# DecaYale/SYN3R

Measured on AMD Instinct MI355X. Metric: llff_3view_train_loop_iters_per_sec, higher is better.
Workload: dtype f32 raster / f16 UNet (f32 accumulate); 1 GPU; LLFF fern-like 3-view block: 50 raster fwd+bwd iters (l1 loss) (200000 Gaussians, 1920x1080, SH3) + 1 SVD (step,pass): CFG UNet fwd [2,14,8,72,128] f16 + fused Euler step; frames=14, parallelism=scene-parallel x1

## Files before the change

### syn3r_amd/csrc/raster_bin.hip

```cpp
#include "common.h"
#include "raster_common.h"

using namespace syn3r;

namespace syn3r {

size_t binning_bytes(long long P) {
    size_t n = (size_t)(P > 0 ? P : 1);
    return 2 * align256(n * 8) + 2 * align256(n * 4) + sort_scratch_bytes(n) + 256;
}

BinningState carve_binning(void* buf, long long P) {
    size_t n = (size_t)(P > 0 ? P : 1);
    char* p = (char*)buf;
    BinningState b;
    b.keys_a = (unsigned long long*)p; p += align256(n * 8);
    b.keys_b = (unsigned long long*)p; p += align256(n * 8);
    b.vals_a = (unsigned*)p; p += align256(n * 4);
    b.vals_b = (unsigned*)p; p += align256(n * 4);
    b.sort_scratch = p;
    return b;
}

}

namespace {

__global__ void __launch_bounds__(256) k_dup_tiles(int N, const unsigned* __restrict__ order,
                                                   const float* __restrict__ means2D, const int* __restrict__ radii,
                                                   const unsigned* __restrict__ offsets, int gx, int gy,
                                                   unsigned* __restrict__ keys, unsigned* __restrict__ vals,
                                                   unsigned cap, unsigned* __restrict__ header,
                                                   uint2* __restrict__ ranges, int tiles) {
    const int i = blockIdx.x * 256 + threadIdx.x;
    for (int t = i; t < tiles; t += gridDim.x * 256) ranges[t] = make_uint2(0u, 0u);
    const int lane = threadIdx.x & 63;
    const bool valid = i < N;
    unsigned id = valid ? order[i] : 0u;
    int r = valid ? radii[id] : 0;
    int x0 = 0, y0 = 0, x1 = 0, y1 = 0;
    if (r > 0) tile_rect(means2D[2 * (size_t)id], means2D[2 * (size_t)id + 1], r, gx, gy, x0, y0, x1, y1);
    const int w = x1 - x0;
    const unsigned cnt = (unsigned)(w * (y1 - y0));
    const unsigned incl = wave_scan_incl(cnt);
    const unsigned local = incl - cnt;
    const unsigned total = __shfl(incl, 63, 64);
    const int first = blockIdx.x * 256 + (threadIdx.x & ~63);
    const unsigned base = first < N ? offsets[first] : 0u;
    const float inv_w = w > 0 ? 1.0f / (float)w : 0.0f;
    for (unsigned t = 0; t < total; t += 64) {
        const unsigned p = t + lane;
        int j = 0;
#pragma unroll
        for (int step = 32; step > 0; step >>= 1) {
            unsigned lc = __shfl(local, j + step, 64);
            if (lc <= p) j += step;
        }
        const unsigned k = p - __shfl(local, j, 64);
        const int xj = __shfl(x0, j, 64), yj = __shfl(y0, j, 64), wj = __shfl(w, j, 64);
        const float iwj = __shfl(inv_w, j, 64);
        const unsigned idj = __shfl(id, j, 64);
        if (p < total) {
            const int ty = (int)(((float)k + 0.5f) * iwj);
            int tyc = ty;
            if ((unsigned)(tyc * wj) > k) --tyc;
            else if ((unsigned)((tyc + 1) * wj) <= k) ++tyc;
            const int tx = (int)k - tyc * wj;
            const unsigned o = base + p;
            if (o < cap) {
                keys[o] = (unsigned)((yj + tyc) * gx + xj + tx);
                vals[o] = idj;
            } else {
                header[1] = 1u;
            }
        }
    }
}

__global__ void __launch_bounds__(256) k_tile_ranges(long long P_cap, const unsigned* __restrict__ header,
                                                     const unsigned* __restrict__ keys,
                                                     uint2* __restrict__ ranges) {
    long long P = (long long)header[0];
    if (P > P_cap) P = P_cap;
    long long i = (long long)blockIdx.x * 256 + threadIdx.x;
    if (i >= P) return;
    unsigned cur = keys[i];
    if (i == 0) ranges[cur].x = 0;
    else {
        unsigned prev = keys[i - 1];
        if (cur != prev) {
            ranges[prev].y = (unsigned)i;
            ranges[cur].x = (unsigned)i;
        }
    }
    if (i == P - 1) ranges[cur].y = (unsigned)P;
}

constexpr int kBinThreads = 512;
constexpr int kOffThreads = 1024;
#ifndef SYN3R_MAX_SUPER
#define SYN3R_MAX_SUPER 512
#endif
constexpr int kMaxSuper = SYN3R_MAX_SUPER;

struct BinPlan { int ss, sgx, sgy, nsuper, rounds, nchunks; bool ok; };
inline BinPlan bin_plan(int N, int gx, int gy) {
    BinPlan b;
    for (b.ss = 0; b.ss <= 3; ++b.ss) {
        const int side = 1 << b.ss;
        b.sgx = (gx + side - 1) / side; b.sgy = (gy + side - 1) / side;
        b.nsuper = b.sgx * b.sgy;
        if (b.nsuper <= kMaxSuper) break;
    }
    if (b.ss > 3) b.ss = 3;
    b.ok = b.nsuper <= kMaxSuper;
    const int max_chunks = b.ok ? (int)(kBinCounters / (size_t)b.nsuper) : 1;
    const int units = (N + kBinThreads - 1) / kBinThreads;
    b.rounds = (units + max_chunks - 1) / max_chunks;
    if (b.rounds < 1) b.rounds = 1;
    b.nchunks = (units + b.rounds - 1) / b.rounds;
    return b;
}

inline bool hier_binning(int N, int gx, int gy) {
    static const int on = tune_env("SYN3R_BIN_HIER", 1);
    return on != 0 && bin_plan(N, gx, gy).ok;
}

struct BinRect { int x0, y0, x1, y1; };
__device__ __forceinline__ BinRect bin_rect(int i, int N, const float* __restrict__ means2D, const int* __restrict__ radii, int gx, int gy) {
    BinRect r; r.x0 = r.y0 = r.x1 = r.y1 = 0;
    if (i < N) {
        const int rad = radii[i];
        if (rad > 0) tile_rect(means2D[2 * (size_t)i], means2D[2 * (size_t)i + 1], rad, gx, gy, r.x0, r.y0, r.x1, r.y1);
    }
    return r;
}
__device__ __forceinline__ unsigned short clip_rect(const BinRect& q, int sx, int sy, int ss) {
    const int bx = sx << ss, by = sy << ss, side = 1 << ss;
    const int rx0 = max(q.x0 - bx, 0), rx1 = min(q.x1 - bx, side), ry0 = max(q.y0 - by, 0), ry1 = min(q.y1 - by, side);
    return (unsigned short)(rx0 | (rx1 << 4) | (ry0 << 8) | (ry1 << 12));
}

__global__ void __launch_bounds__(kBinThreads) k_super_count(int N, const float* __restrict__ means2D, const int* __restrict__ radii,
                                                             int gx, int gy, int ss, int sgx, int nsuper, int rounds, int nchunks,
                                                             unsigned* __restrict__ counters, unsigned* __restrict__ header) {
    __shared__ unsigned tot[kMaxSuper];
    for (int s = threadIdx.x; s < nsuper; s += kBinThreads) tot[s] = 0u;
    __syncthreads();
    int pairs = 0;
    for (int r = 0; r < rounds; ++r) {
        const int i = (blockIdx.x * rounds + r) * kBinThreads + threadIdx.x;
        const BinRect q = bin_rect(i, N, means2D, radii, gx, gy);
        if (q.x1 > q.x0 && q.y1 > q.y0) {
            pairs += (q.x1 - q.x0) * (q.y1 - q.y0);
            const int side1 = (1 << ss) - 1, sx0 = q.x0 >> ss, sx1 = (q.x1 + side1) >> ss, sy0 = q.y0 >> ss, sy1 = (q.y1 + side1) >> ss;
            for (int sy = sy0; sy < sy1; ++sy)
                for (int sx = sx0; sx < sx1; ++sx) atomicAdd(&tot[sy * sgx + sx], 1u);
        }
    }
    __syncthreads();
    for (int s = threadIdx.x; s < nsuper; s += kBinThreads) counters[(size_t)blockIdx.x * nsuper + s] = tot[s];
    __shared__ unsigned pairs_s;
    if (threadIdx.x == 0) pairs_s = 0u;
    __syncthreads();
    pairs = wave_sum_i(pairs);
    if ((threadIdx.x & 63) == 0 && pairs) atomicAdd(&pairs_s, (unsigned)pairs);
    __syncthreads();
    if (threadIdx.x == 0 && pairs_s) atomicAdd(&header[3], pairs_s);
}

__global__ void __launch_bounds__(kBinThreads) k_super_append(int N, const float* __restrict__ depths, const float* __restrict__ means2D,
                                                              const int* __restrict__ radii, int gx, int gy, int ss, int sgx, int nsuper,
                                                              int rounds, int nchunks, const unsigned* __restrict__ counters,
                                                              unsigned* __restrict__ sstart, unsigned cap,
                                                              unsigned long long* __restrict__ skeys, unsigned* __restrict__ header) {
    __shared__ unsigned run[kMaxSuper];
    __shared__ unsigned tot_s[kMaxSuper], pre_s[kMaxSuper];
    __shared__ unsigned part_tot[kMaxSuper > kBinThreads ? kMaxSuper : kBinThreads], part_pre[kMaxSuper > kBinThreads ? kMaxSuper : kBinThreads];
    const int lane = threadIdx.x & 63, wv = threadIdx.x >> 6;
    {
        const int PARTS = max(1, min(8, kBinThreads / nsuper));
        const int per = (nchunks + PARTS - 1) / PARTS;
        for (int w = threadIdx.x; w < nsuper * PARTS; w += kBinThreads) {
            const int s_ = w % nsuper, part = w / nsuper;
            const int c0 = part * per, c1 = min(nchunks, c0 + per);
            unsigned tot = 0, pre = 0;
            constexpr int UN = 32;
            for (int cb = c0; cb < c1; cb += UN) {
                unsigned c[UN];
#pragma unroll
                for (int u = 0; u < UN; ++u) c[u] = cb + u < c1 ? counters[(size_t)(cb + u) * nsuper + s_] : 0u;
#pragma unroll
                for (int u = 0; u < UN; ++u) { tot += c[u]; pre += cb + u < (int)blockIdx.x ? c[u] : 0u; }
            }
            part_tot[w] = tot; part_pre[w] = pre;
        }
        __syncthreads();
        for (int s_ = threadIdx.x; s_ < nsuper; s_ += kBinThreads) {
            unsigned tot = 0, pre = 0;
            for (int k = 0; k < PARTS; ++k) { tot += part_tot[k * nsuper + s_]; pre += part_pre[k * nsuper + s_]; }
            tot_s[s_] = tot; pre_s[s_] = pre;
        }
        __syncthreads();
        if (wv == 0) {
            constexpr int PER = kMaxSuper / 64;
            unsigned c[PER], sum = 0;
#pragma unroll
            for (int k = 0; k < PER; ++k) { const int s_ = lane * PER + k; c[k] = s_ < nsuper ? tot_s[s_] : 0u; sum += c[k]; }
            const unsigned incl = wave_scan_incl(sum);
            unsigned ex = incl - sum;
#pragma unroll
            for (int k = 0; k < PER; ++k) {
                const int s_ = lane * PER + k;
                if (s_ < nsuper) {
                    run[s_] = ex + pre_s[s_];
                    if (blockIdx.x == 0) sstart[s_] = ex;
                }
                ex += c[k];
            }
            if (blockIdx.x == 0 && lane == 63) { sstart[nsuper] = incl; header[2] = incl; }
        }
        __syncthreads();
    }
    for (int r = 0; r < rounds; ++r) {
        const int i = (blockIdx.x * rounds + r) * kBinThreads + threadIdx.x;
        const BinRect q = bin_rect(i, N, means2D, radii, gx, gy);
        if (q.x1 > q.x0 && q.y1 > q.y0) {
            const unsigned long long key = ((unsigned long long)__float_as_uint(depths[i]) << 32) | (unsigned)i;
            const int side1 = (1 << ss) - 1, sx0 = q.x0 >> ss, sx1 = (q.x1 + side1) >> ss, sy0 = q.y0 >> ss, sy1 = (q.y1 + side1) >> ss;
            for (int sy = sy0; sy < sy1; ++sy)
                for (int sx = sx0; sx < sx1; ++sx) {
                    const unsigned o = atomicAdd(&run[sy * sgx + sx], 1u);
                    if (o < cap) skeys[o] = key;
                    else header[1] = 1u;
                }
        }
    }
}

__device__ __forceinline__ void super_range(int s, const unsigned* __restrict__ sstart, unsigned cap, unsigned& b, unsigned& e) {
    b = min(sstart[s], cap); e = min(sstart[s + 1], cap);
}

constexpr int kSortLds = 4096;
constexpr int kSuperSortThreads = 1024;
__device__ __forceinline__ void cmpx(unsigned long long& a, unsigned long long& b) { if (a > b) { const unsigned long long t = a; a = b; b = t; } }
__device__ __forceinline__ int pair_lo(int t, int j) { return (t << 1) - (t & (j - 1)); }
__device__ __forceinline__ void bitonic_dists(unsigned long long* buf, int m, int j) {
    for (; j >= 2; j >>= 2) {
        const int jh = j >> 1;
        for (int t = threadIdx.x; t < (m >> 2); t += kSuperSortThreads) {
            const int e0 = pair_lo(pair_lo(t, jh), j);
            unsigned long long a = buf[e0], b = buf[e0 + jh], c = buf[e0 + j], d = buf[e0 + j + jh];
            cmpx(a, c); cmpx(b, d);
            cmpx(a, b); cmpx(c, d);
            buf[e0] = a; buf[e0 + jh] = b; buf[e0 + j] = c; buf[e0 + j + jh] = d;
        }
        __syncthreads();
    }
    if (j == 1) {
        for (int t = threadIdx.x; t < (m >> 1); t += kSuperSortThreads) cmpx(buf[2 * t], buf[2 * t + 1]);
        __syncthreads();
    }
}
__device__ __forceinline__ void bitonic_merge(unsigned long long* buf, int m, int k) {
    if (k == 2) {
        for (int t = threadIdx.x; t < (m >> 1); t += kSuperSortThreads) cmpx(buf[2 * t], buf[2 * t + 1]);
        __syncthreads();
        return;
    }
    const int q = k >> 2;
    for (int t = threadIdx.x; t < (m >> 2); t += kSuperSortThreads) {
        const int off = t & (q - 1), blk = (t - off) << 2;
        const int ia = blk + off, ib = ia + q, ird = blk + (k - 1 - off), irc = ird - q;
        unsigned long long a = buf[ia], b = buf[ib], c = buf[irc], d = buf[ird];
        cmpx(a, d); cmpx(b, c);
        cmpx(a, b); cmpx(c, d);
        buf[ia] = a; buf[ib] = b; buf[irc] = c; buf[ird] = d;
    }
    __syncthreads();
    bitonic_dists(buf, m, q >> 1);
}

__device__ __forceinline__ bool rect_has(unsigned r, int rx, int ry) {
    return rx >= (int)(r & 15u) && rx < (int)((r >> 4) & 15u) && ry >= (int)((r >> 8) & 15u) && ry < (int)(r >> 12);
}

constexpr int kBinUnroll = 8;
__device__ __forceinline__ void tile_quarter(unsigned b, unsigned e, int q, unsigned& qb, unsigned& qe) {
    const unsigned len = (e - b + 3u) / 4u;
    qb = min(e, b + (unsigned)q * len); qe = min(e, qb + len);
}

__device__ __forceinline__ void super_tile_counts(int sx, int sy, int ss, int gx, int gy, unsigned n, const unsigned short* srect_b,
                                                  unsigned* __restrict__ tcount) {
    const int lane = threadIdx.x & 63, wv = threadIdx.x >> 6, side = 1 << ss;
    const unsigned len = (n + 3u) / 4u;
    for (int it = wv; it < side * side * 4; it += kSuperSortThreads / 64) {
        const int ti = it >> 2, q = it & 3;
        const int rx = ti & (side - 1), ry = ti >> ss;
        const int tx = (sx << ss) + rx, ty = (sy << ss) + ry;
        if (tx >= gx || ty >= gy) continue;
        const unsigned lo = min(n, (unsigned)q * len), hi = min(n, lo + len);
        unsigned cnt = 0;
        for (unsigned i0 = lo; i0 < hi; i0 += 256) {
            unsigned short r[4];
#pragma unroll
            for (int u = 0; u < 4; ++u) r[u] = srect_b[min(i0 + u * 64 + lane, hi - 1u)];
#pragma unroll
            for (int u = 0; u < 4; ++u) cnt += (i0 + u * 64 + lane < hi && rect_has(r[u], rx, ry)) ? 1u : 0u;
        }
#pragma unroll
        for (int o = 32; o > 0; o >>= 1) cnt += __shfl_xor(cnt, o, 64);
        if (lane == 0) tcount[4 * ((size_t)ty * gx + tx) + q] = cnt;
    }
}

__global__ void __launch_bounds__(kSuperSortThreads, 8) k_super_sort(int N, const float* __restrict__ means2D, const int* __restrict__ radii,
                                                                  int gx, int gy, int ss, int sgx, const unsigned* __restrict__ sstart, unsigned cap,
                                                                  unsigned long long* __restrict__ skeys, unsigned* __restrict__ sid,
                                                                  unsigned short* __restrict__ srect, unsigned* __restrict__ tcount) {
    extern __shared__ __attribute__((aligned(16))) unsigned long long sk[];
    const int s_ = blockIdx.x, sx = s_ % sgx, sy = s_ / sgx;
    unsigned b, e;
    super_range(s_, sstart, cap, b, e);
    const int n = (int)(e - b);
    if (n == 0) { super_tile_counts(sx, sy, ss, gx, gy, 0u, srect, tcount); return; }
    unsigned long long* gk = skeys + b;
    const unsigned long long INF = ~0ull;
    int m = 1;
    while (m < n) m <<= 1;
    const unsigned long long* sorted;
    if (m <= kSortLds) {
        for (int i = threadIdx.x; i < m; i += kSuperSortThreads) sk[i] = i < n ? gk[i] : INF;
        __syncthreads();
        for (int k = 2; k <= m; k <<= 1) bitonic_merge(sk, m, k);
        sorted = sk;
    } else {
        for (int p0 = 0; p0 < n; p0 += kSortLds) {
            for (int i = threadIdx.x; i < kSortLds; i += kSuperSortThreads) sk[i] = p0 + i < n ? gk[p0 + i] : INF;
            __syncthreads();
            for (int k = 2; k <= kSortLds; k <<= 1) bitonic_merge(sk, kSortLds, k);
            for (int i = threadIdx.x; i < kSortLds; i += kSuperSortThreads) if (p0 + i < n) gk[p0 + i] = sk[i];
            __syncthreads();
        }
        for (int k = kSortLds << 1; k <= m; k <<= 1) {
            const int h = k >> 1;
            for (int t = threadIdx.x; t < (m >> 1); t += kSuperSortThreads) {
                const int off = t & (h - 1), l = pair_lo(t, h), r = l - off + (k - 1 - off);
                if (r < n) { unsigned long long a = gk[l], c = gk[r]; if (a > c) { gk[l] = c; gk[r] = a; } }
            }
            __syncthreads();
            for (int j = k >> 2; j >= kSortLds; j >>= 1) {
                for (int t = threadIdx.x; t < (m >> 1); t += kSuperSortThreads) {
                    const int l = pair_lo(t, j), r = l + j;
                    if (r < n) { unsigned long long a = gk[l], c = gk[r]; if (a > c) { gk[l] = c; gk[r] = a; } }
                }
                __syncthreads();
            }
            for (int p0 = 0; p0 < n; p0 += kSortLds) {
                for (int i = threadIdx.x; i < kSortLds; i += kSuperSortThreads) sk[i] = p0 + i < n ? gk[p0 + i] : INF;
                __syncthreads();
                bitonic_dists(sk, kSortLds, kSortLds >> 1);
                for (int i = threadIdx.x; i < kSortLds; i += kSuperSortThreads) if (p0 + i < n) gk[p0 + i] = sk[i];
                __syncthreads();
            }
        }
        sorted = gk;
    }
    if (sorted == sk) {
        unsigned short clip[kSortLds / kSuperSortThreads];
#pragma unroll
        for (int u = 0; u < kSortLds / kSuperSortThreads; ++u) {
            const int i = threadIdx.x + u * kSuperSortThreads;
            clip[u] = 0;
            if (i < n) {
                const unsigned id = (unsigned)sk[i];
                const BinRect q = bin_rect((int)id, N, means2D, radii, gx, gy);
                clip[u] = clip_rect(q, sx, sy, ss);
                sid[b + i] = id;
                srect[b + i] = clip[u];
            }
        }
        __syncthreads();
        unsigned short* sr = (unsigned short*)sk;
#pragma unroll
        for (int u = 0; u < kSortLds / kSuperSortThreads; ++u) {
            const int i = threadIdx.x + u * kSuperSortThreads;
            if (i < n) sr[i] = clip[u];
        }
        __syncthreads();
        super_tile_counts(sx, sy, ss, gx, gy, (unsigned)n, sr, tcount);
        return;
    }
    for (int i = threadIdx.x; i < n; i += kSuperSortThreads) {
        const unsigned id = (unsigned)sorted[i];
        const BinRect q = bin_rect((int)id, N, means2D, radii, gx, gy);
        sid[b + i] = id;
        srect[b + i] = clip_rect(q, sx, sy, ss);
    }
    __syncthreads();
    super_tile_counts(sx, sy, ss, gx, gy, (unsigned)n, srect + b, tcount);
}

__global__ void __launch_bounds__(kOffThreads) k_tile_offsets(int tiles, const unsigned* __restrict__ tcount, unsigned cap,
                                                              uint2* __restrict__ ranges, unsigned* __restrict__ header,
                                                              unsigned* __restrict__ tile_order) {
    __shared__ unsigned smem[kOffThreads / 64 + 1];
    __shared__ unsigned bh[256];
    if (tile_order) { for (int k = threadIdx.x; k < 256; k += kOffThreads) bh[k] = 0u; __syncthreads(); }
    constexpr int PER = 8;
    unsigned carry = 0;
    for (int start = 0; start < tiles; start += kOffThreads * PER) {
        const int t0 = start + threadIdx.x * PER;
        unsigned c[PER], sum = 0;
#pragma unroll
        for (int k = 0; k < PER; ++k) {
            c[k] = 0u;
            if (t0 + k < tiles) { const uint4 q4 = ((const uint4*)tcount)[t0 + k]; c[k] = (q4.x + q4.y) + (q4.z + q4.w); }
            sum += c[k];
        }
        unsigned total;
        unsigned ex = block_exclusive_scan<kOffThreads / 64>(sum, smem, total) + carry;
#pragma unroll
        for (int k = 0; k < PER; ++k) {
            if (t0 + k < tiles) ranges[t0 + k] = c[k] ? make_uint2(min(ex, cap), min(ex + c[k], cap)) : make_uint2(0u, 0u);
            if (tile_order && t0 + k < tiles) atomicAdd(&bh[255u - min(255u, c[k] >> 5)], 1u);
            ex += c[k];
        }
        carry += total;
    }
    if (tile_order) {
        __syncthreads();
        if (threadIdx.x < 64) {
            const int l = threadIdx.x;
            unsigned c[4], sum = 0;
#pragma unroll
            for (int k = 0; k < 4; ++k) { c[k] = bh[4 * l + k]; sum += c[k]; }
            unsigned ex = wave_scan_incl(sum) - sum;
#pragma unroll
            for (int k = 0; k < 4; ++k) { bh[4 * l + k] = ex; ex += c[k]; }
        }
        __syncthreads();
        for (int t = threadIdx.x; t < tiles; t += kOffThreads) {
            const uint4 q4 = ((const uint4*)tcount)[t];
            const unsigned c = (q4.x + q4.y) + (q4.z + q4.w);
            tile_order[atomicAdd(&bh[255u - min(255u, c >> 5)], 1u)] = (unsigned)t;
        }
    }
    if (threadIdx.x == 0) {
        const bool over = carry > cap || header[2] > cap;
        header[0] = over ? max(carry, max(header[3], header[2])) : carry;
        if (over) header[1] = 1u;
    }
}

__global__ void __launch_bounds__(256) k_tile_write(int gx, int tiles, int ss, int sgx, const unsigned* __restrict__ sstart, unsigned cap,
                                                    const unsigned* __restrict__ sid, const unsigned short* __restrict__ srect,
                                                    const uint2* __restrict__ ranges, const unsigned* __restrict__ tcount,
                                                    unsigned* __restrict__ point_list) {
    const int t = blockIdx.x, q = threadIdx.x >> 6, lane = threadIdx.x & 63;
    const int tx = t % gx, ty = t / gx;
    unsigned b, e;
    super_range((ty >> ss) * sgx + (tx >> ss), sstart, cap, b, e);
    tile_quarter(b, e, q, b, e);
    const int rx = tx & ((1 << ss) - 1), ry = ty & ((1 << ss) - 1);
    const unsigned long long lt = (1ull << lane) - 1ull;
    const uint4 q4 = ((const uint4*)tcount)[t];
    unsigned pos = ranges[t].x + (q > 0 ? q4.x : 0u) + (q > 1 ? q4.y : 0u) + (q > 2 ? q4.z : 0u);
    for (unsigned i0 = b; i0 < e; i0 += 64 * kBinUnroll) {
        unsigned short r[kBinUnroll];
        unsigned id[kBinUnroll];
#pragma unroll
        for (int u = 0; u < kBinUnroll; ++u) {
            const unsigned i = i0 + u * 64 + lane;
            r[u] = i < e ? srect[i] : (unsigned short)0;
            id[u] = i < e ? sid[i] : 0u;
        }
#pragma unroll
        for (int u = 0; u < kBinUnroll; ++u) {
            const bool hit = rect_has(r[u], rx, ry);
            const unsigned long long m = __ballot(hit);
            if (hit) {
                const unsigned o = pos + (unsigned)__popcll(m & lt);
                if (o < cap) point_list[o] = id[u];
            }
            pos += (unsigned)__popcll(m);
        }
    }
}

int bits_for(unsigned v) { int b = 0; while (v) { ++b; v >>= 1; } return b; }

}

namespace syn3r {

bool raster_tiles_ordered(int N, int gx, int gy) {
    static const int order_env = tune_env("SYN3R_TILE_ORDER", 1);
    return order_env != 0 && hier_binning(N, gx, gy);
}

int raster_bin_prepare(const GeomState& g, int N, int gx, int gy, bool want_count, hipStream_t stream) {
    if (!hier_binning(N, gx, gy)) {
        int in_b = 0;
        int rc = argsort_depth_u32(g.dkeys_a, g.order_a, g.dkeys_b, g.order_b, (size_t)N, g.sort_scratch, stream, &in_b);
        if (rc) return rc;
        if ((in_b ? g.order_b : g.order_a) != g.order) { set_error("raster_preprocess: unexpected argsort parity"); return SYN3R_E_INVALID; }
        return exclusive_scan_u32(g.tiles_touched, g.point_offsets, (size_t)N, g.header, g.scan_scratch, stream, g.order);
    }
    if (want_count) return exclusive_scan_u32(g.tiles_touched, g.point_offsets, (size_t)N, g.header, g.scan_scratch, stream);
    return SYN3R_OK;
}

int raster_bin_lists(const GeomState& g, const ImageState& im, const BinningState& bn, const int* radii, int N, int gx, int gy,
                     long long P, hipStream_t stream, unsigned** point_list_out, const unsigned** tile_order_out) {
    const size_t tiles = (size_t)gx * gy;
    unsigned* point_list = bn.vals_a;
    unsigned* tile_order = nullptr;
    if (P == 0) {
        if (int rc = check_hip(hipMemsetAsync(im.ranges, 0, tiles * 8, stream), "memset ranges")) return rc;
    } else if (hier_binning(N, gx, gy)) {
        SYN3R_REQUIRE(P < (1ll << 30), "raster_render: pair capacity %lld: the super-tile sort indexes a list with 31-bit integers (2^30 pairs at most)", P);
        const BinPlan bp = bin_plan(N, gx, gy);
        unsigned* counters = im.bin_counters;
        unsigned* sid = bn.vals_b;
        unsigned short* srect = (unsigned short*)bn.keys_a;
        unsigned* sstart = counters + kBinCounters;
        unsigned long long* skeys = bn.keys_b;
        static DevOnce once;
        if (int rc = set_max_lds(once, (const void*)k_super_sort, kSortLds * 8, "hipFuncSetAttribute(super_sort)")) return rc;
        SYN3R_LAUNCH(k_super_count, dim3(bp.nchunks), dim3(kBinThreads), 0, stream, N, (const float*)g.means2D, radii, gx, gy, bp.ss, bp.sgx,
                     bp.nsuper, bp.rounds, bp.nchunks, counters, g.header);
        SYN3R_LAUNCH(k_super_append, dim3(bp.nchunks), dim3(kBinThreads), 0, stream, N, (const float*)g.depths, (const float*)g.means2D, radii,
                     gx, gy, bp.ss, bp.sgx, bp.nsuper, bp.rounds, bp.nchunks, (const unsigned*)counters, sstart, (unsigned)P, skeys, g.header);
        SYN3R_LAUNCH(k_super_sort, dim3(bp.nsuper), dim3(kSuperSortThreads), kSortLds * 8, stream, N, (const float*)g.means2D, radii, gx, gy,
                     bp.ss, bp.sgx, (const unsigned*)sstart, (unsigned)P, skeys, sid, srect, im.tile_counts);
        if (raster_tiles_ordered(N, gx, gy)) tile_order = im.tile_order;
        SYN3R_LAUNCH(k_tile_offsets, dim3(1), dim3(kOffThreads), 0, stream, (int)tiles, (const unsigned*)im.tile_counts, (unsigned)P,
                     im.ranges, g.header, tile_order);
        SYN3R_LAUNCH(k_tile_write, dim3((unsigned)tiles), dim3(256), 0, stream, gx, (int)tiles, bp.ss, bp.sgx,
                     (const unsigned*)sstart, (unsigned)P, (const unsigned*)sid, (const unsigned short*)srect,
                     (const uint2*)im.ranges, (const unsigned*)im.tile_counts, point_list);
    } else {
        unsigned* tk_a = (unsigned*)bn.keys_a;
        unsigned* tk_b = (unsigned*)bn.keys_b;
        SYN3R_LAUNCH(k_dup_tiles, dim3(ceil_div(N, 256)), dim3(256), 0, stream, N, g.order, g.means2D, radii,
                           g.point_offsets, gx, gy, tk_a, bn.vals_a, (unsigned)P, g.header, im.ranges, (int)tiles);
        int in_b = 0;
        int rc = sort_pairs_by_tile_u32(tk_a, bn.vals_a, tk_b, bn.vals_b, (size_t)P, bits_for((unsigned)tiles - 1),
                                        bn.sort_scratch, stream, &in_b, g.header);
        if (rc) return rc;
        const unsigned* keys = in_b ? tk_b : tk_a;
        point_list = in_b ? bn.vals_b : bn.vals_a;
        SYN3R_LAUNCH(k_tile_ranges, dim3(ceil_div(P, 256)), dim3(256), 0, stream, P, g.header, keys, im.ranges);
    }
    *point_list_out = point_list;
    *tile_order_out = tile_order;
    return SYN3R_OK;
}

}
```

### syn3r_amd/csrc/raster_common.h

```cpp
#pragma once
#include <hip/hip_runtime.h>
#include <stdint.h>
#include <stddef.h>

namespace syn3r {

constexpr int kTileX = 16;
constexpr int kTileY = 16;
constexpr int kTilePix = kTileX * kTileY;
constexpr float kNearClip = 0.2f;
constexpr float kFovGuard = 1.3f;
constexpr float kLowPass = 0.3f;
constexpr float kMipFloor = 0.000025f;
constexpr float kAlphaMin = 1.0f / 255.0f;
constexpr float kAlphaMax = 0.99f;
constexpr float kTransmittanceMin = 1e-4f;
constexpr float kLog2e = 1.4426950408889634f;

struct alignas(16) Splat {
    float x, y;
    float cxx, cxy, cyy;
    float opacity;
    float r, g, b;
    float depth;
    float pad0, pad1;
};
static_assert(sizeof(Splat) == 48, "Splat must be 48 bytes");

struct GeomState {
    unsigned* header;
    float* depths;
    float* means2D;
    float* cov3D;
    float* conic_opacity;
    float* rgb;
    unsigned* clamped;
    unsigned* tiles_touched;
    unsigned* point_offsets;
    Splat* splats;
    unsigned* dkeys_a;
    unsigned* dkeys_b;
    unsigned* order_a;
    unsigned* order_b;
    unsigned* order;
    void* sort_scratch;
    void* scan_scratch;
};

#ifndef SYN3R_BIN_COUNTERS
#define SYN3R_BIN_COUNTERS 65536
#endif
constexpr size_t kBinCounters = SYN3R_BIN_COUNTERS;
constexpr size_t kMaxSuperSlots = 4096;
struct ImageState {
    uint2* ranges;
    unsigned* n_contrib;
    float* final_T;
    unsigned* tile_counts;
    unsigned* bin_counters;
    unsigned* tile_order;
};

struct BinningState {
    unsigned long long* keys_a;
    unsigned long long* keys_b;
    unsigned* vals_a;
    unsigned* vals_b;
    void* sort_scratch;
};

inline size_t align256(size_t x) { return (x + 255) & ~(size_t)255; }

size_t scan_scratch_bytes(size_t n);
size_t sort_scratch_bytes(size_t n);
int exclusive_scan_u32(const unsigned* in, unsigned* out, size_t n, unsigned* total_out, void* scratch,
                       hipStream_t stream, const unsigned* perm = nullptr);
int argsort_depth_u32(unsigned* keys_a, unsigned* vals_a, unsigned* keys_b, unsigned* vals_b, size_t n, void* scratch,
                      hipStream_t stream, int* result_in_b);
int sort_pairs_by_tile_u32(unsigned* keys_a, unsigned* vals_a, unsigned* keys_b, unsigned* vals_b, size_t n, int nbits,
                           void* scratch, hipStream_t stream, int* result_in_b, const unsigned* n_dev);
int radix_sort_pairs(unsigned long long* keys_a, unsigned* vals_a, unsigned long long* keys_b, unsigned* vals_b,
                     size_t n, int nbits, void* scratch, hipStream_t stream, int* result_in_b,
                     const unsigned* n_dev = nullptr);

struct Camera {
    float view[16];
    float proj[16];
    float campos[3];
    float tanfovx, tanfovy, focal_x, focal_y;
    int H, W, grid_x, grid_y;
};

size_t geom_bytes(int N);
bool raster_tiles_ordered(int N, int gx, int gy);
size_t image_bytes(int H, int W);
size_t binning_bytes(long long P);
GeomState carve_geom(void* buf, int N);
void raster_fill_camera(Camera& cam, const float* view, const float* proj, const float* campos, float tanfovx, float tanfovy, int H, int W);
ImageState carve_image(void* buf, int H, int W);
BinningState carve_binning(void* buf, long long P);

struct RasterScene {
    int N, sh_degree, sh_coeffs;
    const float *means3D, *scales, *rotations, *opacities, *shs, *confidence;
    float scale_modifier;
    const float *viewmatrix, *projmatrix, *campos;
    float tanfovx, tanfovy;
    int H, W, raw, flags;
    const float* filter3d;
};
inline RasterScene raster_scene(int N, int sh_degree, int sh_coeffs, const float* means3D, const float* scales,
                                const float* rotations, const float* opacities, const float* shs, const float* confidence,
                                float scale_modifier, const float* viewmatrix, const float* projmatrix, const float* campos,
                                float tanfovx, float tanfovy, int H, int W, int raw, int flags, const float* filter3d) {
    return RasterScene{N, sh_degree, sh_coeffs, means3D, scales, rotations, opacities, shs, confidence, scale_modifier,
                       viewmatrix, projmatrix, campos, tanfovx, tanfovy, H, W, raw, flags, filter3d};
}
int raster_check_scene(const char* who, const RasterScene& s);

int raster_bin_prepare(const GeomState& g, int N, int gx, int gy, bool want_count, hipStream_t stream);
int raster_bin_lists(const GeomState& g, const ImageState& im, const BinningState& bn, const int* radii, int N, int gx, int gy,
                     long long P, hipStream_t stream, unsigned** point_list, const unsigned** tile_order);

#ifdef __HIPCC__
__device__ __forceinline__ bool splat_reaches_rect(float mx, float my, float A, float B, float C, float op, float x0,
                                                   float x1, float y0, float y1) {
    if (!(A > 0.0f && C > 0.0f)) return true;
    const float thr = 2.0f * __logf(255.0f * op);
    const float dx0 = x0 - mx, dx1 = x1 - mx, dy0 = y0 - my, dy1 = y1 - my;
    const bool inx = dx0 <= 0.0f && dx1 >= 0.0f, iny = dy0 <= 0.0f && dy1 >= 0.0f;
    float qmin = 0.0f;
    if (!(inx && iny)) {
        qmin = 3.0e38f;
        if (!inx) {
            const float dx = dx0 > 0.0f ? dx0 : dx1;
            const float dy = fminf(fmaxf(-B * dx / C, dy0), dy1);
            qmin = A * dx * dx + 2.0f * B * dx * dy + C * dy * dy;
        }
        if (!iny) {
            const float dy = dy0 > 0.0f ? dy0 : dy1;
            const float dx = fminf(fmaxf(-B * dy / A, dx0), dx1);
            qmin = fminf(qmin, A * dx * dx + 2.0f * B * dx * dy + C * dy * dy);
        }
    }
    return qmin <= thr + (1.0e-3f + 1.0e-4f * thr);
}

__device__ __forceinline__ void tile_rect(float px, float py, int radius, int gx, int gy, int& x0, int& y0, int& x1,
                                          int& y1) {
    x0 = min(gx, max(0, (int)((px - radius) / kTileX)));
    y0 = min(gy, max(0, (int)((py - radius) / kTileY)));
    x1 = min(gx, max(0, (int)((px + radius + kTileX - 1) / kTileX)));
    y1 = min(gy, max(0, (int)((py + radius + kTileY - 1) / kTileY)));
}

typedef float f2 __attribute__((ext_vector_type(2)));
__device__ __forceinline__ f2 splat2(float s) { return (f2){s, s}; }
constexpr int kBlendThreads = 128;
struct BlendFrame {
    int px, py0, py1;
    bool in0, in1;
    float fx;
    f2 fy;
};
struct BlendHalf { float sx0, sx1, sy0, sy1; };
__device__ __forceinline__ BlendFrame blend_frame(unsigned tile, int wq, int lane, int H, int W, int gx) {
    const int tx = tile % gx, ty = tile / gx;
    const int lx = lane & 15, ly = wq * 8 + (lane >> 4);
    BlendFrame f;
    f.px = tx * kTileX + lx; f.py0 = ty * kTileY + ly; f.py1 = f.py0 + 4;
    f.in0 = f.px < W && f.py0 < H; f.in1 = f.px < W && f.py1 < H;
    f.fx = (float)f.px;
    f.fy = (f2){(float)f.py0, (float)f.py1};
    return f;
}
__device__ __forceinline__ BlendHalf blend_half(unsigned tile, int wq, int gx) {
    const int tx = tile % gx, ty = tile / gx;
    BlendHalf h;
    h.sx0 = (float)(tx * kTileX); h.sx1 = h.sx0 + 15.0f;
    h.sy0 = (float)(ty * kTileY + wq * 8); h.sy1 = h.sy0 + 7.0f;
    return h;
}
__device__ __forceinline__ void stage_splat(float4* sm, int slot, const float4& n0, const float4& n1, const float4& n2) {
    sm[slot * 3 + 0] = n0;
    sm[slot * 3 + 1] = n1;
    sm[slot * 3 + 2] = n2;
}
struct BlendEval { float dx; f2 dy, power, G; };
__device__ __forceinline__ BlendEval blend_eval(const float4& a, const float4& b, const BlendFrame& f) {
    BlendEval e;
    e.dx = a.x - f.fx;
    e.dy = splat2(a.y) - f.fy;
    const float hxx = -0.5f * a.z * e.dx * e.dx, bxy = a.w * e.dx;
    e.power = (-0.5f * b.x) * e.dy * e.dy - bxy * e.dy + hxx;
    const f2 pl = e.power * kLog2e;
    e.G = (f2){__builtin_amdgcn_exp2f(pl.x), __builtin_amdgcn_exp2f(pl.y)};
    return e;
}

constexpr float SH_C0 = 0.28209479177387814f;
constexpr float SH_C1 = 0.4886025119029199f;
static __constant__ float SH_C2[5] = {1.0925484305920792f, -1.0925484305920792f, 0.31539156525252005f,
                                      -1.0925484305920792f, 0.5462742152960396f};
static __constant__ float SH_C3[7] = {-0.5900435899266435f, 2.890611442640554f, -0.4570457994644658f, 0.3731763325901154f,
                                      -0.4570457994644658f, 1.445305721320277f, -0.5900435899266435f};
__device__ __forceinline__ float3 xf43(const float* m, float3 p) {
    return make_float3(m[0] * p.x + m[4] * p.y + m[8] * p.z + m[12], m[1] * p.x + m[5] * p.y + m[9] * p.z + m[13],
                       m[2] * p.x + m[6] * p.y + m[10] * p.z + m[14]);
}
__device__ __forceinline__ float4 xf44(const float* m, float3 p) {
    return make_float4(m[0] * p.x + m[4] * p.y + m[8] * p.z + m[12], m[1] * p.x + m[5] * p.y + m[9] * p.z + m[13],
                       m[2] * p.x + m[6] * p.y + m[10] * p.z + m[14], m[3] * p.x + m[7] * p.y + m[11] * p.z + m[15]);
}
struct Rot3 { float R00, R01, R02, R10, R11, R12, R20, R21, R22; };
__device__ __forceinline__ Rot3 quat_rotation(float4 q) {
    const float qr = q.x, qx = q.y, qy = q.z, qz = q.w;
    Rot3 o;
    o.R00 = 1.f - 2.f * (qy * qy + qz * qz); o.R01 = 2.f * (qx * qy - qr * qz); o.R02 = 2.f * (qx * qz + qr * qy);
    o.R10 = 2.f * (qx * qy + qr * qz); o.R11 = 1.f - 2.f * (qx * qx + qz * qz); o.R12 = 2.f * (qy * qz - qr * qx);
    o.R20 = 2.f * (qx * qz - qr * qy); o.R21 = 2.f * (qy * qz + qr * qx); o.R22 = 1.f - 2.f * (qx * qx + qy * qy);
    return o;
}
struct EwaRows { float tx, ty, T00, T01, T02, T10, T11, T12; };
__device__ __forceinline__ EwaRows ewa_rows(const Camera& cam, float t_x, float t_y, float t_z) {
    const float limx = kFovGuard * cam.tanfovx, limy = kFovGuard * cam.tanfovy;
    EwaRows o;
    o.tx = fminf(limx, fmaxf(-limx, t_x / t_z)) * t_z;
    o.ty = fminf(limy, fmaxf(-limy, t_y / t_z)) * t_z;
    const float J00 = cam.focal_x / t_z, J02 = -(cam.focal_x * o.tx) / (t_z * t_z);
    const float J11 = cam.focal_y / t_z, J12 = -(cam.focal_y * o.ty) / (t_z * t_z);
    const float* v = cam.view;
    o.T00 = J00 * v[0] + J02 * v[2]; o.T01 = J00 * v[4] + J02 * v[6]; o.T02 = J00 * v[8] + J02 * v[10];
    o.T10 = J11 * v[1] + J12 * v[2]; o.T11 = J11 * v[5] + J12 * v[6]; o.T12 = J11 * v[9] + J12 * v[10];
    return o;
}
struct EwaCov { float a0, a1, a2, b0, b1, b2, xx, yy, xy; };
__device__ __forceinline__ EwaCov ewa_cov(const EwaRows& w, float c0, float c1, float c2, float c3, float c4, float c5) {
    EwaCov o;
    o.a0 = c0 * w.T00 + c1 * w.T01 + c2 * w.T02; o.a1 = c1 * w.T00 + c3 * w.T01 + c4 * w.T02; o.a2 = c2 * w.T00 + c4 * w.T01 + c5 * w.T02;
    o.b0 = c0 * w.T10 + c1 * w.T11 + c2 * w.T12; o.b1 = c1 * w.T10 + c3 * w.T11 + c4 * w.T12; o.b2 = c2 * w.T10 + c4 * w.T11 + c5 * w.T12;
    o.xx = w.T00 * o.a0 + w.T01 * o.a1 + w.T02 * o.a2;
    o.yy = w.T10 * o.b0 + w.T11 * o.b1 + w.T12 * o.b2;
    o.xy = w.T00 * o.b0 + w.T01 * o.b1 + w.T02 * o.b2;
    return o;
}
__device__ __forceinline__ float mip_rho(float r) { return sqrtf(fmaxf(r, kMipFloor)); }
__device__ __forceinline__ float mip_ratio(float a, float b, float c) {
    const float bb = __fmul_rn(b, b);
    const float d0 = __fmaf_rn(a, c, -bb);
    const float d1 = __fmaf_rn(__fadd_rn(a, kLowPass), __fadd_rn(c, kLowPass), -bb);
    return __fdiv_rn(d0, d1);
}

struct F3dScales { float q0, q1, q2, r0, r1, r2, coef, ff; };
__device__ __forceinline__ F3dScales f3d_scales(float s0, float s1, float s2, float f) {
    F3dScales o;
    o.ff = __fmul_rn(f, f);
    o.q0 = sqrtf(__fmaf_rn(s0, s0, o.ff)); o.q1 = sqrtf(__fmaf_rn(s1, s1, o.ff)); o.q2 = sqrtf(__fmaf_rn(s2, s2, o.ff));
    o.r0 = o.q0 > 0.0f ? __fdiv_rn(s0, o.q0) : 1.0f;
    o.r1 = o.q1 > 0.0f ? __fdiv_rn(s1, o.q1) : 1.0f;
    o.r2 = o.q2 > 0.0f ? __fdiv_rn(s2, o.q2) : 1.0f;
    o.coef = __fmul_rn(__fmul_rn(o.r0, o.r1), o.r2);
    return o;
}
__device__ __forceinline__ float mode_factors(float x, float coef, float rho) { return x * coef * rho; }

#ifdef SYN3R_RASTER_STATS
#define RASTER_STAT(arr, i, n) do { if (lane == 0) atomicAdd(&arr[i], (unsigned long long)(n)); } while (0)
#else
#define RASTER_STAT(arr, i, n)
#endif
#endif

}
```

Before: 413.2 iters/s.

## Replace bitonic super-tile sort with LDS merge sort and merge-path global merges

Per-super-tile depth sorting switches from bitonic networks to a merge sort. Tiles above a size threshold are sorted in LDS with 4-element merge-path steps, and oversized super-tiles are merged in global memory using merge-path splits and a ping-pong buffer (new keys_c). The goal is to cut the O(n log^2 n) compare-exchange work and the many global passes of the bitonic fallback. In exchange it doubles the LDS per block, which may lower occupancy, and adds a scratch key buffer.

```diff
diff --git a/syn3r_amd/csrc/raster_bin.hip b/syn3r_amd/csrc/raster_bin.hip
--- a/syn3r_amd/csrc/raster_bin.hip
+++ b/syn3r_amd/csrc/raster_bin.hip
@@ -7,7 +7,7 @@
 
 size_t binning_bytes(long long P) {
     size_t n = (size_t)(P > 0 ? P : 1);
-    return 2 * align256(n * 8) + 2 * align256(n * 4) + sort_scratch_bytes(n) + 256;
+    return 3 * align256(n * 8) + 2 * align256(n * 4) + align256(sort_scratch_bytes(n)) + 256;
 }
 
 BinningState carve_binning(void* buf, long long P) {
@@ -18,7 +18,8 @@
     b.keys_b = (unsigned long long*)p; p += align256(n * 8);
     b.vals_a = (unsigned*)p; p += align256(n * 4);
     b.vals_b = (unsigned*)p; p += align256(n * 4);
-    b.sort_scratch = p;
+    b.sort_scratch = p; p += align256(sort_scratch_bytes(n));
+    b.keys_c = (unsigned long long*)p;
     return b;
 }
 
@@ -317,83 +318,152 @@
     }
 }
 
+template <typename P>
+__device__ __forceinline__ int merge_split(P A, int la, P B, int lb, int d, int steps) {
+    int lo = max(0, d - lb), hi = min(d, la);
+    for (int s = 0; s < steps; ++s) {
+        if (lo < hi) {
+            const int mid = (lo + hi) >> 1;
+            if (A[mid] <= B[d - 1 - mid]) lo = mid + 1; else hi = mid;
+        }
+    }
+    return lo;
+}
+__device__ __forceinline__ void merge_quad(const unsigned long long* src, unsigned long long* dst, int a0, int la, int b0, int lb, int d, int steps) {
+    const unsigned long long INF = ~0ull;
+    const int i = merge_split(src + a0, la, src + b0, lb, d, steps), j = d - i;
+    unsigned long long a[4], c[4];
+#pragma unroll
+    for (int u = 0; u < 4; ++u) {
+        a[u] = i + u < la ? src[a0 + i + u] : INF;
+        c[u] = j + u < lb ? src[b0 + j + u] : INF;
+    }
+    int ra[4] = {0, 1, 2, 3}, rc[4] = {4, 5, 6, 7};
+#pragma unroll
+    for (int u = 0; u < 4; ++u)
+#pragma unroll
+        for (int v = 0; v < 4; ++v) { const int lt = c[v] < a[u] ? 1 : 0; ra[u] += lt; rc[v] -= lt; }
+    const int room = min(4, la + lb - d);
+#pragma unroll
+    for (int u = 0; u < 4; ++u) {
+        if (ra[u] < room) dst[d + ra[u]] = a[u];
+        if (rc[u] < room) dst[d + rc[u]] = c[u];
+    }
+}
+__device__ __forceinline__ unsigned long long* lds_merge_sort(unsigned long long* s0, unsigned long long* s1,
+                                                              const unsigned long long* __restrict__ g, int cnt) {
+    const int t = threadIdx.x, nq = (cnt + 3) >> 2, np = nq << 2;
+    if (t < nq) {
+        unsigned long long k[4];
+#pragma unroll
+        for (int u = 0; u < 4; ++u) k[u] = 4 * t + u < cnt ? g[4 * t + u] : ~0ull;
+        cmpx(k[0], k[1]); cmpx(k[2], k[3]); cmpx(k[0], k[2]); cmpx(k[1], k[3]); cmpx(k[1], k[2]);
+#pragma unroll
+        for (int u = 0; u < 4; ++u) s0[4 * t + u] = k[u];
+    }
+    __syncthreads();
+    int steps = 3;
+    for (int L = 4; L < np; L <<= 1, ++steps) {
+        if (t < nq) {
+            const int o = 4 * t, base = o & ~(2 * L - 1);
+            const int la = min(L, np - base), lb = min(L, np - base - la);
+            merge_quad(s0, s1 + base, base, la, base + la, lb, o - base, steps);
+        }
+        __syncthreads();
+        unsigned long long* x = s0; s0 = s1; s1 = x;
+    }
+    return s0;
+}
+
+constexpr int kSortMergeMin = 513;
+constexpr int kSplitSlots = 1024;
+
 __global__ void __launch_bounds__(kSuperSortThreads, 8) k_super_sort(int N, const float* __restrict__ means2D, const int* __restrict__ radii,
                                                                   int gx, int gy, int ss, int sgx, const unsigned* __restrict__ sstart, unsigned cap,
-                                                                  unsigned long long* __restrict__ skeys, unsigned* __restrict__ sid,
-                                                                  unsigned short* __restrict__ srect, unsigned* __restrict__ tcount) {
+                                                                  unsigned long long* __restrict__ skeys, unsigned long long* __restrict__ skeys2,
+                                                                  unsigned* __restrict__ sid, unsigned short* __restrict__ srect,
+                                                                  unsigned* __restrict__ tcount, int merge_min) {
     extern __shared__ __attribute__((aligned(16))) unsigned long long sk[];
-    const int s_ = blockIdx.x, sx = s_ % sgx, sy = s_ / sgx;
+    unsigned long long* s0 = sk;
+    unsigned long long* s1 = sk + kSortLds;
+    const int s_ = blockIdx.x;
+    const int sx = s_ % sgx, sy = s_ / sgx;
     unsigned b, e;
     super_range(s_, sstart, cap, b, e);
     const int n = (int)(e - b);
     if (n == 0) { super_tile_counts(sx, sy, ss, gx, gy, 0u, srect, tcount); return; }
     unsigned long long* gk = skeys + b;
     const unsigned long long INF = ~0ull;
-    int m = 1;
-    while (m < n) m <<= 1;
-    const unsigned long long* sorted;
-    if (m <= kSortLds) {
-        for (int i = threadIdx.x; i < m; i += kSuperSortThreads) sk[i] = i < n ? gk[i] : INF;
-        __syncthreads();
-        for (int k = 2; k <= m; k <<= 1) bitonic_merge(sk, m, k);
-        sorted = sk;
-    } else {
-        for (int p0 = 0; p0 < n; p0 += kSortLds) {
-            for (int i = threadIdx.x; i < kSortLds; i += kSuperSortThreads) sk[i] = p0 + i < n ? gk[p0 + i] : INF;
+    if (n <= kSortLds) {
+        const unsigned long long* sorted;
+        if (n < merge_min) {
+            int m = 1;
+            while (m < n) m <<= 1;
+            for (int i = threadIdx.x; i < m; i += kSuperSortThreads) s0[i] = i < n ? gk[i] : INF;
             __syncthreads();
-            for (int k = 2; k <= kSortLds; k <<= 1) bitonic_merge(sk, kSortLds, k);
-            for (int i = threadIdx.x; i < kSortLds; i += kSuperSortThreads) if (p0 + i < n) gk[p0 + i] = sk[i];
-            __syncthreads();
-        }
-        for (int k = kSortLds << 1; k <= m; k <<= 1) {
-            const int h = k >> 1;
-            for (int t = threadIdx.x; t < (m >> 1); t += kSuperSortThreads) {
-                const int off = t & (h - 1), l = pair_lo(t, h), r = l - off + (k - 1 - off);
-                if (r < n) { unsigned long long a = gk[l], c = gk[r]; if (a > c) { gk[l] = c; gk[r] = a; } }
+            for (int k = 2; k <= m; k <<= 1) bitonic_merge(s0, m, k);
+            sorted = s0;
+        } else {
+            sorted = lds_merge_sort(s0, s1, gk, n);
+        }
+        unsigned short* sr = (unsigned short*)(sorted == s0 ? s1 : s0);
+#pragma unroll
+        for (int u = 0; u < kSortLds / kSuperSortThreads; ++u) {
+            const int i = threadIdx.x + u * kSuperSortThreads;
+            if (i < n) {
+                const unsigned id = (unsigned)sorted[i];
+                const BinRect q = bin_rect((int)id, N, means2D, radii, gx, gy);
+                const unsigned short clip = clip_rect(q, sx, sy, ss);
+                sid[b + i] = id;
+                srect[b + i] = clip;
+                sr[i] = clip;
+            }
+        }
+        __syncthreads();
+        super_tile_counts(sx, sy, ss, gx, gy, (unsigned)n, sr, tcount);
+        return;
+    }
+    unsigned long long* ga = gk;
+    unsigned long long* gb = skeys2 + b;
+    for (int p0 = 0; p0 < n; p0 += kSortLds) {
+        const int cnt = min(kSortLds, n - p0);
+        const unsigned long long* s = lds_merge_sort(s0, s1, ga + p0, cnt);
+        for (int i = threadIdx.x; i < cnt; i += kSuperSortThreads) ga[p0 + i] = s[i];
+        __syncthreads();
+    }
+    __shared__ int split_s[kSplitSlots];
+    const int ntiles = (n + kSortLds - 1) / kSortLds;
+    int steps = 13;
+    for (int L = kSortLds; L < n; L <<= 1, ++steps) {
+        for (int k0 = 0; k0 < ntiles; k0 += kSplitSlots / 2) {
+            const int k1 = min(ntiles, k0 + kSplitSlots / 2);
+            {
+                const int k = k0 + ((int)threadIdx.x >> 1);
+                if (k < k1) {
+                    const int o = k * kSortLds, base = o & ~(2 * L - 1);
+                    const int la = min(L, n - base), lb = min(L, n - base - la);
+                    const int d = min(o - base + ((int)threadIdx.x & 1) * kSortLds, la + lb);
+                    split_s[threadIdx.x] = merge_split((const unsigned long long*)ga + base, la, (const unsigned long long*)ga + base + la, lb, d, steps);
+                }
             }
             __syncthreads();
-            for (int j = k >> 2; j >= kSortLds; j >>= 1) {
-                for (int t = threadIdx.x; t < (m >> 1); t += kSuperSortThreads) {
-                    const int l = pair_lo(t, j), r = l + j;
-                    if (r < n) { unsigned long long a = gk[l], c = gk[r]; if (a > c) { gk[l] = c; gk[r] = a; } }
-                }
+            for (int k = k0; k < k1; ++k) {
+                const int o = k * kSortLds, base = o & ~(2 * L - 1);
+                const int la = min(L, n - base), lb = min(L, n - base - la);
+                const int d0 = o - base, d1 = min(d0 + kSortLds, la + lb);
+                const int i0 = split_s[2 * (k - k0)], i1 = split_s[2 * (k - k0) + 1];
+                const int j0 = d0 - i0, ac = i1 - i0, len = d1 - d0, bc = len - ac;
+                for (int i = threadIdx.x; i < len; i += kSuperSortThreads) s0[i] = i < ac ? ga[base + i0 + i] : ga[base + la + j0 + (i - ac)];
                 __syncthreads();
+                if (4 * (int)threadIdx.x < len) merge_quad(s0, s1, 0, ac, ac, bc, 4 * (int)threadIdx.x, 13);
+                __syncthreads();
+                for (int i = threadIdx.x; i < len; i += kSuperSortThreads) gb[o + i] = s1[i];
             }
-            for (int p0 = 0; p0 < n; p0 += kSortLds) {
-                for (int i = threadIdx.x; i < kSortLds; i += kSuperSortThreads) sk[i] = p0 + i < n ? gk[p0 + i] : INF;
-                __syncthreads();
-                bitonic_dists(sk, kSortLds, kSortLds >> 1);
-                for (int i = threadIdx.x; i < kSortLds; i += kSuperSortThreads) if (p0 + i < n) gk[p0 + i] = sk[i];
-                __syncthreads();
-            }
-        }
-        sorted = gk;
-    }
-    if (sorted == sk) {
-        unsigned short clip[kSortLds / kSuperSortThreads];
-#pragma unroll
-        for (int u = 0; u < kSortLds / kSuperSortThreads; ++u) {
-            const int i = threadIdx.x + u * kSuperSortThreads;
-            clip[u] = 0;
-            if (i < n) {
-                const unsigned id = (unsigned)sk[i];
-                const BinRect q = bin_rect((int)id, N, means2D, radii, gx, gy);
-                clip[u] = clip_rect(q, sx, sy, ss);
-                sid[b + i] = id;
-                srect[b + i] = clip[u];
-            }
-        }
-        __syncthreads();
-        unsigned short* sr = (unsigned short*)sk;
-#pragma unroll
-        for (int u = 0; u < kSortLds / kSuperSortThreads; ++u) {
-            const int i = threadIdx.x + u * kSuperSortThreads;
-            if (i < n) sr[i] = clip[u];
-        }
-        __syncthreads();
-        super_tile_counts(sx, sy, ss, gx, gy, (unsigned)n, sr, tcount);
-        return;
-    }
+            __syncthreads();
+        }
+        unsigned long long* x = ga; ga = gb; gb = x;
+    }
+    const unsigned long long* sorted = ga;
     for (int i = threadIdx.x; i < n; i += kSuperSortThreads) {
         const unsigned id = (unsigned)sorted[i];
         const BinRect q = bin_rect((int)id, N, means2D, radii, gx, gy);
@@ -530,13 +600,14 @@
         unsigned* sstart = counters + kBinCounters;
         unsigned long long* skeys = bn.keys_b;
         static DevOnce once;
-        if (int rc = set_max_lds(once, (const void*)k_super_sort, kSortLds * 8, "hipFuncSetAttribute(super_sort)")) return rc;
+        if (int rc = set_max_lds(once, (const void*)k_super_sort, 2 * kSortLds * 8, "hipFuncSetAttribute(super_sort)")) return rc;
+        static const int merge_min = tune_env("SYN3R_SORT_MERGE_MIN", kSortMergeMin);
         SYN3R_LAUNCH(k_super_count, dim3(bp.nchunks), dim3(kBinThreads), 0, stream, N, (const float*)g.means2D, radii, gx, gy, bp.ss, bp.sgx,
                      bp.nsuper, bp.rounds, bp.nchunks, counters, g.header);
         SYN3R_LAUNCH(k_super_append, dim3(bp.nchunks), dim3(kBinThreads), 0, stream, N, (const float*)g.depths, (const float*)g.means2D, radii,
                      gx, gy, bp.ss, bp.sgx, bp.nsuper, bp.rounds, bp.nchunks, (const unsigned*)counters, sstart, (unsigned)P, skeys, g.header);
-        SYN3R_LAUNCH(k_super_sort, dim3(bp.nsuper), dim3(kSuperSortThreads), kSortLds * 8, stream, N, (const float*)g.means2D, radii, gx, gy,
-                     bp.ss, bp.sgx, (const unsigned*)sstart, (unsigned)P, skeys, sid, srect, im.tile_counts);
+        SYN3R_LAUNCH(k_super_sort, dim3(bp.nsuper), dim3(kSuperSortThreads), 2 * kSortLds * 8, stream, N, (const float*)g.means2D, radii, gx, gy,
+                     bp.ss, bp.sgx, (const unsigned*)sstart, (unsigned)P, skeys, bn.keys_c, sid, srect, im.tile_counts, merge_min);
         if (raster_tiles_ordered(N, gx, gy)) tile_order = im.tile_order;
         SYN3R_LAUNCH(k_tile_offsets, dim3(1), dim3(kOffThreads), 0, stream, (int)tiles, (const unsigned*)im.tile_counts, (unsigned)P,
                      im.ranges, g.header, tile_order);
diff --git a/syn3r_amd/csrc/raster_common.h b/syn3r_amd/csrc/raster_common.h
--- a/syn3r_amd/csrc/raster_common.h
+++ b/syn3r_amd/csrc/raster_common.h
@@ -67,6 +67,7 @@
     unsigned* vals_a;
     unsigned* vals_b;
     void* sort_scratch;
+    unsigned long long* keys_c;
 };
 
 inline size_t align256(size_t x) { return (x + 255) & ~(size_t)255; }
```

Result: no change. 415.7 iters/s (median of 6 runs) (+0.6%).
